# facebookresearch/LaViLa

Measured on AMD Instinct MI355X. Metric: clip-text pairs/s (whole node), TSF-B/16 4x224^2 + CLIP text tower, fwd+loss+bwd+AdamW (caption bound from the host tokens: INTEGRATION.md 1c one-line driver change; unmodified loop = config.device_readback), higher is better.
Workload: dtype bf16

## Files before the change

### include/lavila_hip.h

```cpp
#ifndef LAVILA_HIP_H
#define LAVILA_HIP_H

#include <stdint.h>

#ifdef __cplusplus
extern "C" {
#endif
#pragma GCC visibility push(default)

enum { LVL_F32 = 0, LVL_BF16 = 1 };
enum { LVL_OK = 0, LVL_EINVAL = -22, LVL_ENOSYS = -38, LVL_EHIP = -5 };
enum { LVL_ATTN_SPACE = 0, LVL_ATTN_TIME = 1, LVL_ATTN_CAUSAL = 2  };
enum { LVL_EPI_BIAS = 0, LVL_EPI_BIAS_QUICKGELU = 1, LVL_EPI_QUICKGELU_BWD = 2, LVL_EPI_BIAS_RESIDUAL = 3,
       LVL_EPI_BIAS_QUICKGELU_DERIV = 4, LVL_EPI_MUL_AUX_COLSUM = 5 };
enum { LVL_ACT_GELU_NEW = 0, LVL_ACT_SQRELU = 1 };

const char* lvl_version(void);
int lvl_debug_late_workgroups(int mod);
int lvl_set_compute_units(int n);
const char* lvl_last_error(void);
int64_t lvl_workspace_floats(const char* op, int64_t rows, int64_t cols);

int lvl_layernorm_fwd(const void* x, const void* x2, const float* xbias, const float* gamma,
                      const float* beta, void* s_out, void* y, float* mean, float* rstd,
                      int64_t rows, int cols, float eps, int dtype, void* stream);
int lvl_layernorm_bwd(const void* dy, const void* x, const void* x2, const float* xbias,
                      const float* gamma, const float* mean, const float* rstd, const void* dadd,
                      void* dx, void* dx_plain, float* dgamma, float* dbeta, float* dxsum, float* ws,
                      int64_t rows, int cols, int dtype, void* stream);

enum { LVL_LN_PLAIN = 1, LVL_LN_GENERAL = 2 };
int lvl_layernorm_fwd_mixed(const float* x, const void* x2, const float* xbias, const float* gamma,
                            const float* beta, float* s_out, void* y, float* mean, float* rstd,
                            int64_t rows, int cols, float eps, int flags, void* stream);
int lvl_layernorm_bwd_mixed(const void* dy, const float* x, const void* x2, const float* xbias,
                            const float* gamma, const float* mean, const float* rstd, const float* dadd,
                            float* dx, void* dx2, float* dgamma, float* dbeta, float* dxsum, float* ws,
                            int64_t rows, int cols, int flags, void* stream);

int lvl_droppath_add_layernorm_fwd(const void* res, const void* y, const float* ybias, const float* scale,
                                   const float* gamma, const float* beta, void* s_out, void* h_out, float* mean,
                                   float* rstd, int64_t rows, int64_t rows_per_sample, int cols, float eps,
                                   int dtype, void* stream);
int lvl_droppath_add_layernorm_bwd(const void* dh, const void* s, const float* gamma, const float* mean,
                                   const float* rstd, const float* scale, const void* dadd, void* ds, void* dy,
                                   float* dgamma, float* dbeta, float* dysum, float* ws, int64_t rows,
                                   int64_t rows_per_sample, int cols, int dtype, void* stream);

int lvl_layernorm_apply(const void* x, const void* x2, const float* xbias, const float* gamma,
                        const float* beta, const float* mean, const float* rstd, void* y,
                        int64_t rows, int cols, int dtype, void* stream);

int lvl_quickgelu_apply(const void* u, void* a, int64_t rows, int cols, int dtype, void* stream);

int lvl_bias_quickgelu_fwd(const void* u, const float* bias, void* a, int64_t rows, int cols,
                           int dtype, void* stream);
int lvl_bias_quickgelu_bwd(const void* da, const void* u, const float* bias, void* du, float* dbias,
                           float* ws, int64_t rows, int cols, int dtype, void* stream);

int lvl_patchify(const float* video, void* patches, int B, int C, int F, int H, int W, int P,
                 int frame_major, int dtype, void* stream);

int lvl_embed_tokens_fwd(const void* pe, const float* cls, const float* pos, const float* temporal,
                         void* x, int B, int F, int N, int D, int dtype, void* stream);
int64_t lvl_embed_tokens_bwd_ws(int F, int N, int D);
int lvl_embed_tokens_bwd(const void* dx, float* dpos, float* dtem, float* ws, int B, int F, int N, int D, int tem_rows,
                         int dtype, void* stream);

int lvl_text_embed_fwd(const int64_t* tokens, int64_t tok_stride, const float* table, const float* pos, void* x, int B,
                       int L, int W, int V, int dtype, void* stream);
int64_t lvl_text_embed_bwd_ws(int B, int L, int V);
int lvl_text_embed_bwd(const void* dx, const int64_t* tokens, int64_t tok_stride, float* dtable, float* dpos, int* ws,
                       int B, int L, int W, int V, int ctx, int dtype, void* stream);

int lvl_divided_attn_fwd(const void* qkv, void* out, float* lse, float* ws, int B, int F, int N,
                         int H, int mode, int dtype, void* stream);
int lvl_divided_attn_bwd(const void* qkv, const void* out, const void* dout, const float* lse,
                         void* dqkv, float* ws, int B, int F, int N, int H, int mode, int dtype,
                         void* stream);

int lvl_attention_fast_path(int mode, int F, int N, int H);
int lvl_attention_fast_path_f32(int mode, int F, int N, int H);
int lvl_debug_f32_generic(int on);
int lvl_debug_space_stream(int mode);
int lvl_debug_stream_variant(int v);
int lvl_set_fp8_qk(int on);
int lvl_debug_generic_attention_calls(int reset);

int lvl_causal_attn_fwd(const void* qkv, void* out, float* lse, int B, int L, int H, int dtype,
                        void* stream);
int lvl_causal_attn_bwd(const void* qkv, const void* out, const void* dout, const float* lse,
                        void* dqkv, float* ws, int B, int L, int H, int dtype, void* stream);

int lvl_clip_loss_fwd(const void* img_all, const void* txt_all, const float* scale, int B, int G,
                      int E, int row0, float* stats, int32_t* argmax, float* logits, int dtype,
                      void* stream);
int lvl_clip_loss_bwd(const void* img_all, const void* txt_all, const float* lse_all,
                      const float* scale, const float* upstream, float coef, int B, int G, int E,
                      int row0, int rows_only, float* dimg, float* dtxt, int dtype, void* stream);

int lvl_ssl_clip_loss_fwd(const void* img_all, const void* txt_all, const int32_t* ind_all,
                          const float* scales3, int B, int G, int E, int row0, float* stats,
                          int32_t* argmax, float* logits, int dtype, void* stream);
int lvl_ssl_clip_loss_bwd(const void* img_all, const void* txt_all, const int32_t* ind_all,
                          const float* lse_all, const float* scales3, const float* upstream, float coef,
                          int B, int G, int E, int row0, float* dimg, float* dtxt, int dtype,
                          void* stream);

int lvl_margin_loss_prepare(const void* img_all, const void* txt_all, const float* weight, float margin, int G,
                            int E, float* prep, int dtype, void* stream);
int lvl_margin_loss_fwd(const void* img_all, const void* txt_all, const float* prep, int B, int G, int E,
                        int row0, int with_diag, float* hinge, int32_t* count, int dtype, void* stream);
int lvl_margin_loss_bwd(const void* img_all, const void* txt_all, const float* prep, const float* upstream,
                        float coef, int B, int G, int E, int row0, float* dimg, float* dtxt, int dtype,
                        void* stream);

int lvl_token_xent_fwd(const void* logits, int64_t row_stride, const int64_t* labels, int64_t label_stride,
                       int64_t rows, int vocab, int64_t pad_id, float* lse, float* nll, int32_t* pred,
                       int32_t* correct, int32_t* counted, int dtype, void* stream);
int lvl_token_xent_reduce(const float* nll, const int32_t* correct, const int32_t* counted, int B, int T,
                          float* out3, void* stream);
int lvl_token_xent_bwd(const void* logits, int64_t row_stride, const int64_t* labels, int64_t label_stride,
                       const float* lse, const float* upstream, float coef, int64_t rows, int vocab, int64_t pad_id,
                       void* dlogits, int dtype, void* stream);

int lvl_cls_attn_fwd(const void* q, const void* kv, void* out, float* lse, int B, int T, int H, int dtype, void* stream);
int lvl_cls_attn_bwd(const void* q, const void* kv, const void* out, const void* dout, const float* lse, float* dq,
                     void* dkv, int B, int T, int H, int dtype, void* stream);

int lvl_mq_cross_attn_fwd(const void* q, int64_t q_batch_stride, const void* kv, void* out, int B, int NQ, int H,
                          int Tk, int dtype, void* stream);
int64_t lvl_mq_cross_attn_bwd_ws(int B, int NQ, int H, int shared_q);
int lvl_mq_cross_attn_bwd(const void* q, int64_t q_batch_stride, const void* kv, const void* dout, void* dq, void* dkv,
                          float* ws, int B, int NQ, int H, int Tk, int dtype, void* stream);

int lvl_linear_skinny(const void* x, const void* w, const float* bias, void* y, int M, int N, int K, int act, void* stream);
int lvl_linear_skinny_f32c(const void* x3, const void* w3, const float* bias, float* y, int M, int N, int K3, int act,
                           void* stream);
int lvl_linear_skinny_ln(const void* res, const void* y, const float* gate, const float* gamma, const float* beta,
                         float eps, void* res_out, const void* w, const float* bias, void* out, int M, int N, int K,
                         int act, void* stream);
int lvl_gpt2_embed(const int64_t* ids, const void* wte, const void* wpe, const int* pos_dev, void* out, int rows, int L,
                   int D, int vocab, int positions, int dtype, void* stream);
int lvl_gated_add_layernorm(const void* res, const void* y, const float* gate, const float* gamma, const float* beta,
                            float eps, void* sum_out, void* h_out, int rows, int D, int dtype, void* stream);
int lvl_act_inplace(void* u, int64_t n, int act, int dtype, void* stream);
int lvl_decode_self_attn(const void* qkv, void* cache, const int* pos_dev, void* out, int B, int Tcap, int H, int dtype,
                         void* stream);
int lvl_cross_attn_rows_fwd(const void* q, const void* kv, void* out, int rows, int qrep, int Tk, int H, int dtype,
                            void* stream);
int lvl_gated_add_layernorm_train(const void* res, const void* y, const float* gate, const float* gamma,
                                  const float* beta, float eps, void* sum_out, void* h_out, float* mean, float* rstd,
                                  int rows, int D, int dtype, void* stream);
int lvl_gated_add_layernorm_bwd(const void* dh, const void* s, const void* y, const float* gate, const float* gamma,
                                const float* mean, const float* rstd, const void* dadd, void* ds, void* dy, float* dgamma,
                                float* dbeta, float* dgate, float* ws, int rows, int D, int dtype, void* stream);
int lvl_act_fwd(const void* u, void* a, int64_t n, int act, int dtype, void* stream);
int lvl_act_bwd(const void* u, const void* da, void* du, int64_t n, int act, int dtype, void* stream);
int lvl_cross_attn_rows_bwd(const void* q, const void* kv, const void* dout, void* dq, void* dkv, int rows, int qrep,
                            int Tk, int H, int dtype, void* stream);

int lvl_sample_max_vocab(void);
int lvl_sample_next_token(const void* logits, int64_t row_stride, int rows, int vocab, float temperature, int top_k,
                          float top_p, const float* uniform, const int64_t* target, int64_t pad_id, int64_t* next_token,
                          float* nll, float* counted, float* dbg, void* stream);

int lvl_linear_tn(const void* x, const void* w, const float* bias, void* y, void* aux_out, const void* aux_in,
                  float* colsum, float* ws, uint32_t* sched, int64_t M, int N, int K, int epilogue, int dtype,
                  void* stream);

int lvl_linear_wgrad(const void* dy, const void* x, float* dw, float* dbias, float* ws, uint32_t* sched, int64_t M,
                     int N, int K, int dtype, void* stream);

int lvl_qkv_bias_grad(const void* dqkv, const void* dout, float* dbias, float* ws, int64_t rows, int D, int dtype,
                      void* stream);
int64_t lvl_divided_attn_bwd_bias_ws(int B, int F, int N, int H, int mode, int dtype);
int lvl_divided_attn_bwd_bias(const void* qkv, const void* out, const void* dout, const float* lse, void* dqkv, float* ws,
                              const float* dout_colsum, float* dbias, float* ws2, int B, int F, int N, int H, int mode,
                              int dtype, void* stream);
int lvl_debug_time_bwd_rider(int mode);
int lvl_vec_mat_f32(const float* v, const float* W, float* out, int N, int K, void* stream);

int lvl_cast_transpose(const float* src, void* dst, void* dst_t, int N, int K, void* stream);
int lvl_cast_transpose_multi(const void* desc, int count, int64_t total_tiles, void* stream);

int lvl_split_bf16x3(const float* src, void* dst, int64_t rows, int cols, int64_t src_row_stride,
                     int64_t dst_row_stride, int64_t dst_term_stride, int role, void* stream);

#pragma GCC visibility pop
#ifdef __cplusplus
}
#endif
#endif
```

### lavila_amd/_cabi.py

```python
import ctypes
import os
import threading

import torch

_HERE = os.path.dirname(os.path.abspath(__file__))
LIB_PATH = os.path.join(_HERE, 'lib', 'liblavila_hip.so')

LVL_F32, LVL_BF16 = 0, 1
ATTN_SPACE, ATTN_TIME = 0, 1
EPI_BIAS, EPI_BIAS_QUICKGELU, EPI_QUICKGELU_BWD, EPI_BIAS_RESIDUAL, EPI_BIAS_QUICKGELU_DERIV, EPI_MUL_AUX_COLSUM = 0, 1, 2, 3, 4, 5
LN_PLAIN, LN_GENERAL = 1, 2
ACT_GELU_NEW, ACT_SQRELU = 0, 1

_c = ctypes
_P, _I, _L, _F = _c.c_void_p, _c.c_int, _c.c_int64, _c.c_float

SIGNATURES = {
    'lvl_version': (_c.c_char_p, []),
    'lvl_set_compute_units': (_I, [_I]),
    'lvl_debug_late_workgroups': (_I, [_I]),
    'lvl_last_error': (_c.c_char_p, []),
    'lvl_workspace_floats': (_L, [_c.c_char_p, _L, _L]),
    'lvl_layernorm_fwd': (_I, [_P, _P, _P, _P, _P, _P, _P, _P, _P, _L, _I, _F, _I, _P]),
    'lvl_layernorm_bwd': (_I, [_P, _P, _P, _P, _P, _P, _P, _P, _P, _P, _P, _P, _P, _P, _L, _I, _I, _P]),
    'lvl_layernorm_fwd_mixed': (_I, [_P, _P, _P, _P, _P, _P, _P, _P, _P, _L, _I, _F, _I, _P]),
    'lvl_layernorm_bwd_mixed': (_I, [_P, _P, _P, _P, _P, _P, _P, _P, _P, _P, _P, _P, _P, _P, _L, _I, _I, _P]),
    'lvl_droppath_add_layernorm_fwd': (_I, [_P] * 10 + [_L, _L, _I, _F, _I, _P]),
    'lvl_droppath_add_layernorm_bwd': (_I, [_P] * 13 + [_L, _L, _I, _I, _P]),
    'lvl_layernorm_apply': (_I, [_P, _P, _P, _P, _P, _P, _P, _P, _L, _I, _I, _P]),
    'lvl_quickgelu_apply': (_I, [_P, _P, _L, _I, _I, _P]),
    'lvl_bias_quickgelu_fwd': (_I, [_P, _P, _P, _L, _I, _I, _P]),
    'lvl_bias_quickgelu_bwd': (_I, [_P, _P, _P, _P, _P, _P, _L, _I, _I, _P]),
    'lvl_patchify': (_I, [_P, _P, _I, _I, _I, _I, _I, _I, _I, _I, _P]),
    'lvl_embed_tokens_fwd': (_I, [_P, _P, _P, _P, _P, _I, _I, _I, _I, _I, _P]),
    'lvl_divided_attn_fwd': (_I, [_P, _P, _P, _P, _I, _I, _I, _I, _I, _I, _P]),
    'lvl_divided_attn_bwd': (_I, [_P, _P, _P, _P, _P, _P, _I, _I, _I, _I, _I, _I, _P]),
    'lvl_attention_fast_path': (_I, [_I, _I, _I, _I]),
    'lvl_attention_fast_path_f32': (_I, [_I, _I, _I, _I]),
    'lvl_debug_f32_generic': (_I, [_I]),
    'lvl_debug_space_stream': (_I, [_I]),
    'lvl_debug_stream_variant': (_I, [_I]),
    'lvl_set_fp8_qk': (_I, [_I]),
    'lvl_debug_generic_attention_calls': (_I, [_I]),
    'lvl_causal_attn_fwd': (_I, [_P, _P, _P, _I, _I, _I, _I, _P]),
    'lvl_causal_attn_bwd': (_I, [_P, _P, _P, _P, _P, _P, _I, _I, _I, _I, _P]),
    'lvl_clip_loss_fwd': (_I, [_P, _P, _P, _I, _I, _I, _I, _P, _P, _P, _I, _P]),
    'lvl_clip_loss_bwd': (_I, [_P, _P, _P, _P, _P, _F, _I, _I, _I, _I, _I, _P, _P, _I, _P]),
    'lvl_ssl_clip_loss_fwd': (_I, [_P, _P, _P, _P, _I, _I, _I, _I, _P, _P, _P, _I, _P]),
    'lvl_ssl_clip_loss_bwd': (_I, [_P, _P, _P, _P, _P, _P, _F, _I, _I, _I, _I, _P, _P, _I, _P]),
    'lvl_margin_loss_prepare': (_I, [_P, _P, _P, _F, _I, _I, _P, _I, _P]),
    'lvl_margin_loss_fwd': (_I, [_P, _P, _P, _I, _I, _I, _I, _I, _P, _P, _I, _P]),
    'lvl_margin_loss_bwd': (_I, [_P, _P, _P, _P, _F, _I, _I, _I, _I, _P, _P, _I, _P]),
    'lvl_token_xent_fwd': (_I, [_P, _L, _P, _L, _L, _I, _L, _P, _P, _P, _P, _P, _I, _P]),
    'lvl_token_xent_reduce': (_I, [_P, _P, _P, _I, _I, _P, _P]),
    'lvl_token_xent_bwd': (_I, [_P, _L, _P, _L, _P, _P, _F, _L, _I, _L, _P, _I, _P]),
    'lvl_linear_tn': (_I, [_P, _P, _P, _P, _P, _P, _P, _P, _P, _L, _I, _I, _I, _I, _P]),
    'lvl_linear_wgrad': (_I, [_P, _P, _P, _P, _P, _P, _L, _I, _I, _I, _P]),
    'lvl_cast_transpose': (_I, [_P, _P, _P, _I, _I, _P]),
    'lvl_cast_transpose_multi': (_I, [_P, _I, _L, _P]),
    'lvl_split_bf16x3': (_I, [_P, _P, _L, _I, _L, _L, _L, _I, _P]),
    'lvl_cls_attn_fwd': (_I, [_P, _P, _P, _P, _I, _I, _I, _I, _P]),
    'lvl_cls_attn_bwd': (_I, [_P, _P, _P, _P, _P, _P, _P, _I, _I, _I, _I, _P]),
    'lvl_mq_cross_attn_fwd': (_I, [_P, _L, _P, _P, _I, _I, _I, _I, _I, _P]),
    'lvl_mq_cross_attn_bwd_ws': (_L, [_I, _I, _I, _I]),
    'lvl_mq_cross_attn_bwd': (_I, [_P, _L, _P, _P, _P, _P, _P, _I, _I, _I, _I, _I, _P]),
    'lvl_qkv_bias_grad': (_I, [_P, _P, _P, _P, _L, _I, _I, _P]),
    'lvl_divided_attn_bwd_bias_ws': (_L, [_I, _I, _I, _I, _I, _I]),
    'lvl_divided_attn_bwd_bias': (_I, [_P, _P, _P, _P, _P, _P, _P, _P, _P, _I, _I, _I, _I, _I, _I, _P]),
    'lvl_vec_mat_f32': (_I, [_P, _P, _P, _I, _I, _P]),
    'lvl_embed_tokens_bwd_ws': (_L, [_I, _I, _I]),
    'lvl_embed_tokens_bwd': (_I, [_P, _P, _P, _P, _I, _I, _I, _I, _I, _I, _P]),
    'lvl_text_embed_fwd': (_I, [_P, _L, _P, _P, _P, _I, _I, _I, _I, _I, _P]),
    'lvl_text_embed_bwd_ws': (_L, [_I, _I, _I]),
    'lvl_text_embed_bwd': (_I, [_P, _P, _L, _P, _P, _P, _I, _I, _I, _I, _I, _I, _P]),
    'lvl_debug_time_bwd_rider': (_I, [_I]),
    'lvl_linear_skinny': (_I, [_P, _P, _P, _P, _I, _I, _I, _I, _P]),
    'lvl_linear_skinny_f32c': (_I, [_P, _P, _P, _P, _I, _I, _I, _I, _P]),
    'lvl_linear_skinny_ln': (_I, [_P, _P, _P, _P, _P, _F, _P, _P, _P, _P, _I, _I, _I, _I, _P]),
    'lvl_sample_max_vocab': (_I, []),
    'lvl_sample_next_token': (_I, [_P, _L, _I, _I, _F, _I, _F, _P, _P, _L, _P, _P, _P, _P, _P]),
    'lvl_gpt2_embed': (_I, [_P, _P, _P, _P, _P, _I, _I, _I, _I, _I, _I, _P]),
    'lvl_gated_add_layernorm': (_I, [_P, _P, _P, _P, _P, _F, _P, _P, _I, _I, _I, _P]),
    'lvl_act_inplace': (_I, [_P, _L, _I, _I, _P]),
    'lvl_gated_add_layernorm_train': (_I, [_P, _P, _P, _P, _P, _F, _P, _P, _P, _P, _I, _I, _I, _P]),
    'lvl_gated_add_layernorm_bwd': (_I, [_P] * 14 + [_I, _I, _I, _P]),
    'lvl_act_fwd': (_I, [_P, _P, _L, _I, _I, _P]),
    'lvl_act_bwd': (_I, [_P, _P, _P, _L, _I, _I, _P]),
    'lvl_cross_attn_rows_bwd': (_I, [_P, _P, _P, _P, _P, _I, _I, _I, _I, _I, _P]),
    'lvl_decode_self_attn': (_I, [_P, _P, _P, _P, _I, _I, _I, _I, _P]),
    'lvl_cross_attn_rows_fwd': (_I, [_P, _P, _P, _I, _I, _I, _I, _I, _P]),
}

_lib = None
_lock = threading.Lock()


class HipExtensionError(RuntimeError):
    pass


def lib():
    global _lib
    if _lib is not None:
        return _lib
    with _lock:
        if _lib is None:
            if not os.path.exists(LIB_PATH):
                raise HipExtensionError(
                    f'{LIB_PATH} is missing: build it with `python -m lavila_amd.build` '
                    '(or __graft_entry__.build()); lavila_amd has no CPU / eager fallback')
            try:
                handle = ctypes.CDLL(LIB_PATH)
            except OSError as e:
                raise HipExtensionError(f'cannot load {LIB_PATH}: {e}') from e
            for name, (res, args) in SIGNATURES.items():
                fn = getattr(handle, name)
                fn.restype = res
                fn.argtypes = args
            cus = os.environ.get('LAVILA_COMPUTE_UNITS')
            if cus and handle.lvl_set_compute_units(int(cus)) != 0:
                raise HipExtensionError('LAVILA_COMPUTE_UNITS: ' + handle.lvl_last_error().decode(errors='replace'))
            _lib = handle
    return _lib


def check(rc, what):
    if rc != 0:
        msg = lib().lvl_last_error().decode(errors='replace')
        raise HipExtensionError(f'{what} failed (status {rc}): {msg}')


def dtype_code(t: torch.Tensor) -> int:
    if t.dtype == torch.float32:
        return LVL_F32
    if t.dtype == torch.bfloat16:
        return LVL_BF16
    raise HipExtensionError(
        f'lavila_amd kernels take float32 or bfloat16 activations, got {t.dtype} '
        '(fp16 autocast is remapped to bf16 by the model wrappers; see INTEGRATION.md)')


def require_device(*tensors):
    cur = None
    for t in tensors:
        if t is None:
            continue
        if t.is_cuda:
            if cur is None:
                cur = torch.cuda.current_device()
            if t.device.index != cur:
                raise HipExtensionError(
                    f'lavila_amd: tensor on {t.device} but the current device is cuda:{cur}; call '
                    'torch.cuda.set_device() (one process per GPU) before running the model')
        if not t.is_cuda:
            raise HipExtensionError(
                'lavila_amd: tensor on %s -- the HIP kernels need a ROCm device tensor; there is no CPU '
                'fallback (the CPU oracle under oracle/ is test infrastructure only)' % t.device)
        if not t.is_contiguous():
            raise HipExtensionError('lavila_amd: non-contiguous tensor passed to a HIP kernel')


def ptr(t):
    return None if t is None else ctypes.c_void_p(t.data_ptr())


def stream_ptr():
    return ctypes.c_void_p(torch.cuda.current_stream().cuda_stream)


def workspace(op: str, rows: int, cols: int, device) -> torch.Tensor:
    n = lib().lvl_workspace_floats(op.encode(), rows, cols)
    if n < 0:
        raise HipExtensionError(f'unknown workspace op {op}')
    return torch.empty(max(int(n), 1), dtype=torch.float32, device=device)
```

### lavila_amd/csrc/gemm_tn_mfma.hip

```cpp
#include <type_traits>

#include "common.h"

int lvl_debug_late_mod();
int lvl_colsum_mid_rows();
int lvl_launch_column_reduce(const float* part, int nparts, int width, int seg, float* mid, float* out0, float* out1,
                             float* out2, hipStream_t st);

#pragma clang diagnostic ignored "-Winline-asm"

typedef __attribute__((ext_vector_type(8))) __bf16 gm_bf16x8;
typedef __attribute__((ext_vector_type(16))) float gm_f32x16;

namespace {

constexpr int BK = 64;
constexpr int TM = 256, TN = 256;
constexpr int SLOT = 128 * 128;
constexpr int NSLOT = 8;
constexpr int BIAS_OFF = NSLOT * SLOT;
constexpr int MBOX_OFF = BIAS_OFF + 4 * 1024;
constexpr int SMEM_B = MBOX_OFF + 64;
constexpr int DYN_MIN_NB = 5;
enum { S_X0 = 0, S_X1 = 1, S_W0 = 2, S_W1 = 3 };

__device__ __forceinline__ gm_f32x16 mfma32(uint4 a, uint4 b, gm_f32x16 c) {
  return __builtin_amdgcn_mfma_f32_32x32x16_bf16(__builtin_bit_cast(gm_bf16x8, a), __builtin_bit_cast(gm_bf16x8, b),
                                                 c, 0, 0, 0);
}

__device__ __forceinline__ float quick_gelu_grad(float u) {
  const float s = sigmoid1702(u);
  return s * (1.f + 1.702f * u * (1.f - s));
}

__device__ __forceinline__ float qgelu_grad1(float y, float r) { return fmaf((1.f - r) * y, 1.702f, r); }

__device__ __forceinline__ uint4 widen_pair(uint2 a, uint2 b) {
  const auto r0 = __builtin_amdgcn_permlane32_swap(a.x, b.x, false, false);
  const auto r1 = __builtin_amdgcn_permlane32_swap(a.y, b.y, false, false);
  return make_uint4(r0[0], r1[0], r0[1], r1[1]);
}

__device__ __forceinline__ void gm_store16(void* p, uint4 v) { *reinterpret_cast<uint4*>(p) = v; }

#ifdef GM_AUDIT
#define GM_AUD_STORE(j) (gm_aud_st += 1u << (8 * (j)))
#define GM_AUD_COLPART() (++gm_aud_cp)
constexpr int GM_AUDIT_CAP = 255;
__device__ __forceinline__ int gm_wave_max(int v) {
#pragma unroll
  for (int m = 32; m >= 1; m >>= 1) v = max(v, __shfl_xor(v, m, 64));
  return v;
}
#else
#define GM_AUD_STORE(j) ((void)0)
#define GM_AUD_COLPART() ((void)0)
#endif

template <int EPI, bool F32O>
__global__ __launch_bounds__(512) void gemm_tn_kernel(const uint16_t* __restrict__ X, const uint16_t* __restrict__ W,
                                                      const float* __restrict__ bias, void* __restrict__ Yv,
                                                      void* __restrict__ aux_out_v,
                                                      const void* __restrict__ aux_in_v,
                                                      float* __restrict__ colpart, int64_t M, int N, int K,
                                                      int tiles_n, int ntiles, unsigned* __restrict__ sched,
                                                      int late_mod) {
  using out_t = std::conditional_t<F32O, float, uint16_t>;
  out_t* __restrict__ const Y = static_cast<out_t*>(Yv);
  out_t* __restrict__ const aux_out = static_cast<out_t*>(aux_out_v);
  const out_t* __restrict__ const aux_in = static_cast<const out_t*>(aux_in_v);
  extern __shared__ __attribute__((aligned(1024))) uint8_t smem[];
  const int tid = threadIdx.x, lane = tid & 63;
  const int wave = __builtin_amdgcn_readfirstlane(tid >> 6);
  const int wm = wave >> 2, wn = wave & 3;
  const int nb = K / BK;
  const int nx = gridDim.x >= 8 ? 8 : 1;
  const int bid = blockIdx.x, xcd = bid % nx, wpx = gridDim.x / nx;
  const int tq = ntiles / nx, tr = ntiles % nx;
  const int cnt = tq + (xcd < tr ? 1 : 0);
  const int xstart = xcd < tr ? xcd * (tq + 1) : tr * (tq + 1) + (xcd - tr) * tq;
  const bool dyn = sched != nullptr;
  if (dyn) __builtin_assume(nb >= DYN_MIN_NB);
  if (!dyn && bid / nx >= cnt) return;
  int my_tiles = dyn ? 0x7fffffff : (cnt - bid / nx + wpx - 1) / wpx;
  int pair_even = xstart + bid / nx, pair_odd = pair_even;
  auto set_pair = [&](int i, int v) { if (i & 1) pair_odd = v; else pair_even = v; };
  auto get_pair = [&](int i) { return (i & 1) ? pair_odd : pair_even; };
  uint32_t pend = 0;
  unsigned* const ctr = sched + xcd;
  uint64_t exec_save;
  auto pull = [&]() {
    if (wave == 0)
      asm volatile("s_mov_b64 %1, exec\n\ts_mov_b64 exec, 1\n\tglobal_atomic_add %0, %2, %3, %4 sc0\n\ts_mov_b64 exec, %1"
                   : "=v"(pend), "=&s"(exec_save) : "v"(0u), "v"(1u), "s"(ctr) : "memory");
  };
  auto publish = [&]() {
    if (wave == 0)
      asm volatile("s_mov_b64 %0, exec\n\ts_mov_b64 exec, 1\n\tds_write_b32 %1, %2\n\ts_mov_b64 exec, %0"
                   : "=&s"(exec_save) : "v"((uint32_t)(uintptr_t)smem + MBOX_OFF), "v"(pend) : "memory");
  };
  auto mailbox = [&]() -> int {
    uint32_t v;
    asm volatile("ds_read_b32 %0, %1\n\ts_waitcnt lgkmcnt(0)" : "=v"(v) : "v"((uint32_t)(uintptr_t)smem + MBOX_OFF) : "memory");
    return __builtin_amdgcn_readfirstlane(v);
  };
  const bool late = dyn && late_mod > 0 && bid % late_mod == 1;
  if (dyn && !late) pull();

  auto decode_tile = [&](int pair, int& tm, int& tn) {
    tm = pair / tiles_n;
    tn = pair - tm * tiles_n;
  };

  uint32_t xrel[4], wrel[2], xclamp;
  {
    const int sub = lane >> 3;
    const int chunk = (lane & 7) ^ ((4 * wave + (sub >> 1)) & 7);
#pragma unroll
    for (int h = 0; h < 2; ++h) {
      const int lr = 8 * (wave + 8 * h) + sub;
#pragma unroll
      for (int q = 0; q < 2; ++q) xrel[q * 2 + h] = (uint32_t)(q * 128 + lr) * (uint32_t)(K * 2) + chunk * 16;
      wrel[h] = (uint32_t)((lr >> 5) * 64 + (lr & 31)) * (uint32_t)(K * 2) + chunk * 16;
    }
    xclamp = (uint32_t)((M - 1) * K * 2) + chunk * 16;
  }
  const uint32_t lds0 = (uint32_t)(uintptr_t)smem;
  int f_i = 0, f_j = 0;
  uint32_t f_xrow;
  const char* f_wbase;
  auto fetch_tile = [&](int i) {
    if (!dyn) set_pair(i, xstart + bid / nx + i * wpx);
    const int pair = __builtin_amdgcn_readfirstlane(get_pair(i));
    int tm, tn;
    decode_tile(pair, tm, tn);
    f_xrow = (uint32_t)tm * (uint32_t)(TM * K * 2);
    f_wbase = reinterpret_cast<const char*>(W) + (int64_t)tn * TN * K * 2;
    if (EPI != 2 && bias != nullptr && wave == 0) {
      const uint32_t m0v = __builtin_amdgcn_readfirstlane(lds0 + BIAS_OFF + (uint32_t)(i & 3) * 1024);
      const uint32_t off = (uint32_t)lane * 16;
      const char* base = reinterpret_cast<const char*>(bias + tn * TN);
      asm volatile("s_mov_b32 m0, %0\n\ts_nop 0\n\tglobal_load_lds_dwordx4 %1, %2" ::"s"(m0v), "v"(off), "s"(base)
                   : "memory", "m0");
    }
  };
  auto fetch_advance = [&]() {
    if (++f_j == nb) {
      if (dyn && f_i + 1 < my_tiles) {
        const int v = mailbox();
        if (v < cnt) {
          set_pair(f_i + 1, xstart + v);
        } else {
          my_tiles = f_i + 1;
        }
      }
      if (f_i + 1 < my_tiles) {
        f_j = 0;
        fetch_tile(++f_i);
      } else {
        f_j = nb - 1;
      }
    }
  };
  auto issue_fill = [&](int type, int par, int h) {
    const char* base = type < S_W0 ? reinterpret_cast<const char*>(X) + (int64_t)f_j * (BK * 2)
                                   : f_wbase + (int64_t)f_j * (BK * 2) + (type == S_W1 ? (int64_t)32 * K * 2 : 0);
    uint32_t off;
    if (type < S_W0) {
      off = xrel[type * 2 + h] + f_xrow;
      off = off < xclamp ? off : xclamp;
    } else {
      off = wrel[h];
    }
    const uint32_t m0v =
// ... 285 lines not shown
#ifdef GM_AUDIT
  int* const audit = reinterpret_cast<int*>(colpart + ((EPI == 2 || EPI == 5) ? (size_t)2 * (ntiles / tiles_n) * N : 0)) +
                     ((size_t)bid * 8 + wave) * (1 + GM_AUDIT_CAP) * 4;
  int aud_n = 0, aud_rec[4] = {0, 0, 0, 0};
#endif
  if (late) {
    my_tiles = 0;
  } else if (dyn) {
    asm volatile("s_waitcnt vmcnt(0)" ::: "memory");
    publish();
    asm volatile("s_waitcnt lgkmcnt(0)" ::: "memory");
    __builtin_amdgcn_s_barrier();
    const int v = mailbox();
    if (v >= cnt) my_tiles = 0;
    pair_even = xstart + v;
    __builtin_amdgcn_s_barrier();
    if (my_tiles) pull();
  }
  GM_STAMP();
  if (my_tiles > 0) {
  fetch_tile(0);
#pragma unroll
  for (int b0 = 0; b0 < 2; ++b0) {
    issue_group(S_X0, b0 * 4);
    issue_group(S_W0, b0 * 4);
    issue_group(S_W1, b0 * 4);
    issue_group(S_X1, b0 * 4);
    fetch_advance();
  }
#define GM_BAR(N)                                                     \
  do {                                                                \
    asm volatile("s_waitcnt vmcnt(%0)" ::"n"(N) : "memory");          \
    __builtin_amdgcn_s_barrier();                                     \
    asm volatile("" ::: "memory");                                    \
    __builtin_amdgcn_sched_barrier(0);                                \
  } while (0)
#define GM_PHASE(xf, wf, c, rd, dm)                                                                       \
  do {                                                                                                    \
    _Pragma("unroll") for (int kk = 0; kk < 4; ++kk) {                                                    \
      _Pragma("unroll") for (int mt = 0; mt < 2; ++mt) {                                                  \
        c[mt] = mfma32(wf[kk], xf[mt * 4 + kk], c[mt]);                                                   \
        __builtin_amdgcn_sched_barrier(0);                                                                \
        rd(kk * 2 + mt);                                                                                  \
        dm(kk * 2 + mt);                                                                                  \
        __builtin_amdgcn_sched_barrier(0);                                                                \
      }                                                                                                   \
    }                                                                                                     \
  } while (0)
  GM_BAR(12);
  read_x(S_X0, xA);
  read_w(S_W0, wA);
  __builtin_amdgcn_sched_barrier(0);
  GM_STAMP();
  init_acc(0);
  constexpr int NS = F32O ? 0 : (EPI == 1 || EPI == 4 ? 32 : 16);
  auto k_block = [&](auto a0_, auto a1_) {
    constexpr int A0 = decltype(a0_)::value, A1 = decltype(a1_)::value;
    const uint8_t* sb = smem + par * SLOT;
    const uint8_t* sbn = smem + (par ^ 4) * SLOT;
    auto rd_w1 = [&](int k) { if (k < 4) wB[k] = *reinterpret_cast<const uint4*>(sb + S_W1 * SLOT + wa[k]); };
    auto rd_x1 = [&](int k) { xB[k] = *reinterpret_cast<const uint4*>(sb + S_X1 * SLOT + xa[k & 3] + (k >> 2) * 4096); };
    auto rd_x0 = [&](int k) { xA[k] = *reinterpret_cast<const uint4*>(sbn + S_X0 * SLOT + xa[k & 3] + (k >> 2) * 4096); };
    auto rd_w0 = [&](int k) { if (k & 1) wA[k >> 1] = *reinterpret_cast<const uint4*>(sbn + S_W0 * SLOT + wa[k >> 1]); };
    auto dm_none = [&](int) {};
    auto dm_x0w0 = [&](int k) {
      if (k == 0) issue_fill(S_X0, par, 0);
      if (k == 2) issue_fill(S_X0, par, 1);
      if (k == 4) issue_fill(S_W0, par, 0);
      if (k == 6) issue_fill(S_W0, par, 1);
    };
    auto dm_w1 = [&](int k) {
      if (k == 1) issue_fill(S_W1, par, 0);
      if (k == 5) issue_fill(S_W1, par, 1);
    };
    auto dm_x1 = [&](int k) {
      if (k == 0) issue_fill(S_X1, par, 0);
      if (k == 4) issue_fill(S_X1, par, 1);
    };
    GM_BAR(10 + A0);
    GM_PHASE(xA, wA, acc[0][0], rd_w1, dm_none);
    GM_BAR(8 + A0);
    GM_PHASE(xA, wB, acc[0][1], rd_x1, dm_x0w0);
    GM_BAR(10 + A1);
    GM_PHASE(xB, wB, acc[1][1], rd_x0, dm_w1);
    GM_BAR(10 + A1);
    GM_PHASE(xB, wA, acc[1][0], rd_w0, dm_x1);
    fetch_advance();
    par ^= 4;
  };
  using I0 = std::integral_constant<int, 0>;
  using IS = std::integral_constant<int, NS>;
  for (int i = 0; i < my_tiles; ++i) {
    int j = 0;
    if (i > 0) {
#ifdef GM_AUDIT
      if (lane == 0 && aud_n < GM_AUDIT_CAP) {
#pragma unroll
        for (int q = 0; q < 4; ++q) audit[4 * (1 + aud_n) + q] = aud_rec[q];
      }
      ++aud_n;
#endif
      k_block(IS{}, IS{});
      if (nb > 1) k_block(IS{}, I0{});
      j = 2;
    }
    for (; j < nb; ++j) {
      if (dyn && j == 2) {
        if (wave == 0) asm volatile("s_waitcnt vmcnt(10)" ::: "memory");
        publish();
      }
      k_block(I0{}, I0{});
    }
    GM_STAMP();
    if (dyn && my_tiles == 0x7fffffff) pull();
    const int pair = get_pair(i);
    int tm, tn;
    decode_tile(pair, tm, tn);
    epilogue(tm, tn, i);
    const bool tail = NS > 0 && __builtin_amdgcn_readfirstlane((int64_t)tm * TM + TM > M ? 1 : 0);
    if (tail) asm volatile("s_waitcnt vmcnt(0)" ::: "memory");
#ifdef GM_AUDIT
    {
      int issued = gm_wave_max((int)gm_aud_cp);
#pragma unroll
      for (int q = 0; q < 4; ++q) issued += gm_wave_max((int)((gm_aud_st >> (8 * q)) & 255u));
      aud_rec[0] = tm;
      aud_rec[1] = tn;
      aud_rec[2] = issued;
      aud_rec[3] = tail ? 0 : NS;
      gm_aud_st = gm_aud_cp = 0;
    }
#endif
    GM_STAMP();
    init_acc(i + 1);
    __builtin_amdgcn_sched_barrier(0);
  }
  }
#undef GM_BAR
#undef GM_PHASE
  asm volatile("s_waitcnt vmcnt(0)" ::: "memory");
#ifdef GM_AUDIT
  if (lane == 0) audit[0] = aud_n;
#endif
  asm volatile("" ::"v"(pend));
  if (dyn && wave == 0 && lane == 0) {
    const unsigned gone = __hip_atomic_fetch_add(sched + 8, 1u, __ATOMIC_RELAXED, __HIP_MEMORY_SCOPE_AGENT);
    if (gone == gridDim.x - 1) {
#pragma unroll
      for (int q = 0; q < 9; ++q) __hip_atomic_store(sched + q, 0u, __ATOMIC_RELAXED, __HIP_MEMORY_SCOPE_AGENT);
    }
  }
}

int num_cus() { return lvl_persistent_cus(); }

template <int EPI, bool F32O = false>
int launch_tn(const void* x, const void* w, const float* bias, void* y, void* aux_out, const void* aux_in,
              float* colpart, int64_t M, int N, int K, unsigned* sched, hipStream_t st) {
  constexpr int shmem = SMEM_B;
  const int rc = lvl_allow_lds<gemm_tn_kernel<EPI, F32O>>();
  if (rc != LVL_OK) return rc;
  const int tiles_n = N / TN;
  const int64_t tiles_m = (M + TM - 1) / TM;
  const int64_t ntiles = tiles_m * tiles_n;
  if (ntiles > 0x7fffffff) return lvl_fail(LVL_EINVAL, "linear_tn: too many tiles");
  int grid = (int)(ntiles < num_cus() ? ntiles : num_cus());
  if (grid >= 8) grid -= grid % 8;
  if (K / BK < DYN_MIN_NB) sched = nullptr;
  hipLaunchKernelGGL((gemm_tn_kernel<EPI, F32O>), dim3((unsigned)grid), dim3(512), shmem, st, (const uint16_t*)x,
                     (const uint16_t*)w, bias, y, aux_out, aux_in, colpart, M,
                     N, K, tiles_n, (int)ntiles, sched, sched ? lvl_debug_late_mod() : 0);
  LVL_CHECK_LAUNCH("linear_tn");
  return LVL_OK;
}

}

int64_t lvl_linear_tn_workspace_floats(int64_t M, int64_t N) {
  return (2 * ((M + TM - 1) / TM) + lvl_colsum_mid_rows()) * N;
}

#ifdef GM_TRACE
extern "C" int lvl_linear_tn_trace(const void* x, const void* w, const float* bias, void* y, void* trace, int64_t M,
                                   int N, int K, void* stream) {
  return launch_tn<0>(x, w, bias, y, nullptr, nullptr, (float*)trace, M, N, K, nullptr, (hipStream_t)stream);
}
extern "C" int lvl_linear_tn_trace_epi(const void* x, const void* w, const float* bias, void* y, void* aux_out,
                                       const void* aux_in, void* trace, int64_t M, int N, int K, int epilogue, void* stream) {
  hipStream_t st = (hipStream_t)stream;
  switch (epilogue) {
    case 0: return launch_tn<0>(x, w, bias, y, nullptr, nullptr, (float*)trace, M, N, K, nullptr, st);
    case 1: return launch_tn<1>(x, w, bias, y, aux_out, nullptr, (float*)trace, M, N, K, nullptr, st);
    case 3: return launch_tn<3>(x, w, bias, y, nullptr, aux_in, (float*)trace, M, N, K, nullptr, st);
    case 4: return launch_tn<4>(x, w, bias, y, aux_out, nullptr, (float*)trace, M, N, K, nullptr, st);
    case 5: return launch_tn<5>(x, w, nullptr, y, nullptr, aux_in, (float*)trace, M, N, K, nullptr, st);
  }
  return -1;
}
#endif

#ifdef GM_AUDIT
extern "C" int lvl_linear_tn_audit_cap() { return GM_AUDIT_CAP; }
extern "C" int lvl_linear_tn_audit(const void* x, const void* w, const float* bias, void* y, void* aux_out,
                                   const void* aux_in, void* audit, uint32_t* sched, int64_t M, int N, int K, int epilogue,
                                   int dtype, void* stream) {
  hipStream_t st = (hipStream_t)stream;
  float* a = (float*)audit;
  if (dtype == LVL_F32) {
    switch (epilogue) {
      case 0: return launch_tn<0, true>(x, w, bias, y, nullptr, nullptr, a, M, N, K, sched, st);
      case 1: return launch_tn<1, true>(x, w, bias, y, aux_out, nullptr, a, M, N, K, sched, st);
      case 2: return launch_tn<2, true>(x, w, nullptr, y, nullptr, aux_in, a, M, N, K, sched, st);
      case 3: return launch_tn<3, true>(x, w, bias, y, nullptr, aux_in, a, M, N, K, sched, st);
    }
    return -1;
  }
  switch (epilogue) {
    case 0: return launch_tn<0>(x, w, bias, y, nullptr, nullptr, a, M, N, K, sched, st);
    case 1: return launch_tn<1>(x, w, bias, y, aux_out, nullptr, a, M, N, K, sched, st);
    case 2: return launch_tn<2>(x, w, nullptr, y, nullptr, aux_in, a, M, N, K, sched, st);
    case 3: return launch_tn<3>(x, w, bias, y, nullptr, aux_in, a, M, N, K, sched, st);
    case 4: return launch_tn<4>(x, w, bias, y, aux_out, nullptr, a, M, N, K, sched, st);
    case 5: return launch_tn<5>(x, w, nullptr, y, nullptr, aux_in, a, M, N, K, sched, st);
  }
  return -1;
}
#endif

extern "C" int lvl_linear_tn(const void* x, const void* w, const float* bias, void* y, void* aux_out,
                             const void* aux_in, float* colsum, float* ws, uint32_t* sched, int64_t M, int N, int K,
                             int epilogue, int dtype, void* stream) {
  LVL_REQUIRE(x && w && y, "linear_tn: null pointer");
  LVL_REQUIRE(dtype == LVL_BF16 || dtype == LVL_F32, "linear_tn: unknown dtype %d", dtype);
  LVL_REQUIRE(M > 0 && N > 0 && K > 0, "linear_tn: empty problem");
  if (N % TN != 0 || K % BK != 0)
    return lvl_fail(LVL_ENOSYS, "linear_tn: no tiling for N=%d K=%d (N %% 256 == 0 and K %% 64 == 0 needed)", N, K);
  if ((uint64_t)M * K * 2 >= (1ull << 32) || (uint64_t)N * K * 2 >= (1ull << 32))
    return lvl_fail(LVL_ENOSYS, "linear_tn: operand larger than 4 GiB (32-bit DMA offsets)");
  LVL_REQUIRE(lvl_aligned16(x) && lvl_aligned16(w) && lvl_aligned16(y) && lvl_aligned16(bias) &&
                  lvl_aligned16(aux_out) && lvl_aligned16(aux_in),
              "linear_tn: pointers must be 16-byte aligned");
  hipStream_t st = (hipStream_t)stream;
  if (dtype == LVL_F32) {
    LVL_REQUIRE(K % (3 * BK) == 0, "linear_tn (f32 class): K = %d is not 3 x a multiple of 64", K);
    switch (epilogue) {
      case LVL_EPI_BIAS:
        return launch_tn<0, true>(x, w, bias, y, nullptr, nullptr, nullptr, M, N, K, sched, st);
      case LVL_EPI_BIAS_QUICKGELU:
        LVL_REQUIRE(aux_out != nullptr, "linear_tn: the QuickGELU epilogue writes the pre-activation to aux_out");
        return launch_tn<1, true>(x, w, bias, y, aux_out, nullptr, nullptr, M, N, K, sched, st);
      case LVL_EPI_BIAS_RESIDUAL:
        LVL_REQUIRE(aux_in != nullptr, "linear_tn: the residual epilogue reads the residual rows from aux_in");
        return launch_tn<3, true>(x, w, bias, y, nullptr, aux_in, nullptr, M, N, K, sched, st);
      case LVL_EPI_QUICKGELU_BWD: {
        LVL_REQUIRE(aux_in != nullptr && colsum != nullptr && ws != nullptr && lvl_aligned16(ws),
                    "linear_tn: the QuickGELU-backward epilogue needs aux_in, colsum and a workspace");
        const int rc = launch_tn<2, true>(x, w, nullptr, y, nullptr, aux_in, ws, M, N, K, sched, st);
        if (rc != LVL_OK) return rc;
        const int P = (int)(2 * ((M + TM - 1) / TM));
        return lvl_launch_column_reduce(ws, P, N, N, ws + (size_t)P * N, colsum, nullptr, nullptr, st);
      }
      case LVL_EPI_BIAS_QUICKGELU_DERIV:
      case LVL_EPI_MUL_AUX_COLSUM:
        return lvl_fail(LVL_ENOSYS, "linear_tn: epilogue %d is a bf16 epilogue (the f32-class mode keeps the pre-activation: "
                                    "LVL_EPI_BIAS_QUICKGELU / LVL_EPI_QUICKGELU_BWD)", epilogue);
      default:
        return lvl_fail(LVL_EINVAL, "linear_tn: unknown epilogue %d", epilogue);
    }
  }
  switch (epilogue) {
    case LVL_EPI_BIAS:
      return launch_tn<0>(x, w, bias, y, nullptr, nullptr, nullptr, M, N, K, sched, st);
    case LVL_EPI_BIAS_QUICKGELU:
      LVL_REQUIRE(aux_out != nullptr, "linear_tn: the QuickGELU epilogue writes the pre-activation to aux_out");
      return launch_tn<1>(x, w, bias, y, aux_out, nullptr, nullptr, M, N, K, sched, st);
    case LVL_EPI_BIAS_RESIDUAL:
      LVL_REQUIRE(aux_in != nullptr, "linear_tn: the residual epilogue reads the residual rows from aux_in");
      return launch_tn<3>(x, w, bias, y, nullptr, aux_in, nullptr, M, N, K, sched, st);
    case LVL_EPI_QUICKGELU_BWD: {
      LVL_REQUIRE(aux_in != nullptr && colsum != nullptr && ws != nullptr && lvl_aligned16(ws),
                  "linear_tn: the QuickGELU-backward epilogue needs aux_in, colsum and a workspace");
      const int rc = launch_tn<2>(x, w, nullptr, y, nullptr, aux_in, ws, M, N, K, sched, st);
      if (rc != LVL_OK) return rc;
      const int P = (int)(2 * ((M + TM - 1) / TM));
      return lvl_launch_column_reduce(ws, P, N, N, ws + (size_t)P * N, colsum, nullptr, nullptr, st);
    }
    case LVL_EPI_BIAS_QUICKGELU_DERIV:
      LVL_REQUIRE(aux_out != nullptr, "linear_tn: the QuickGELU + derivative epilogue writes quickgelu'(u) to aux_out");
      return launch_tn<4>(x, w, bias, y, aux_out, nullptr, nullptr, M, N, K, sched, st);
    case LVL_EPI_MUL_AUX_COLSUM: {
      LVL_REQUIRE(aux_in != nullptr && colsum != nullptr && ws != nullptr && lvl_aligned16(ws),
                  "linear_tn: the multiply-by-aux epilogue needs aux_in, colsum and a workspace");
      const int rc = launch_tn<5>(x, w, nullptr, y, nullptr, aux_in, ws, M, N, K, sched, st);
      if (rc != LVL_OK) return rc;
      const int P = (int)(2 * ((M + TM - 1) / TM));
      return lvl_launch_column_reduce(ws, P, N, N, ws + (size_t)P * N, colsum, nullptr, nullptr, st);
    }
    default:
      return lvl_fail(LVL_EINVAL, "linear_tn: unknown epilogue %d", epilogue);
  }
}
```

Before: 1558.

## Split tail GEMM tiles into quarter sub-tiles to fill idle CUs

Adds a 128x128 sub-tile GEMM kernel for the bias and residual bf16 epilogues, plus a planner that runs full tiles on the persistent kernel and splits the last partial wave (or tiny problems) into four sub-tiles each, so more compute units stay busy. It also splits short-K problems with more tiles than CUs into row chunks of separate launches. The cost is extra kernel launches and lower per-workgroup reuse in the sub-tile path. A plan query entry point is exported.

```diff
diff --git a/include/lavila_hip.h b/include/lavila_hip.h
--- a/include/lavila_hip.h
+++ b/include/lavila_hip.h
@@ -168,6 +168,7 @@
 int lvl_linear_tn(const void* x, const void* w, const float* bias, void* y, void* aux_out, const void* aux_in,
                   float* colsum, float* ws, uint32_t* sched, int64_t M, int N, int K, int epilogue, int dtype,
                   void* stream);
+int lvl_linear_tn_plan(int64_t M, int N, int K, int epilogue, int dtype, int* out);
 
 int lvl_linear_wgrad(const void* dy, const void* x, float* dw, float* dbias, float* ws, uint32_t* sched, int64_t M,
                      int N, int K, int dtype, void* stream);
diff --git a/lavila_amd/_cabi.py b/lavila_amd/_cabi.py
--- a/lavila_amd/_cabi.py
+++ b/lavila_amd/_cabi.py
@@ -56,6 +56,7 @@
     'lvl_token_xent_reduce': (_I, [_P, _P, _P, _I, _I, _P, _P]),
     'lvl_token_xent_bwd': (_I, [_P, _L, _P, _L, _P, _P, _F, _L, _I, _L, _P, _I, _P]),
     'lvl_linear_tn': (_I, [_P, _P, _P, _P, _P, _P, _P, _P, _P, _L, _I, _I, _I, _I, _P]),
+    'lvl_linear_tn_plan': (_I, [_L, _I, _I, _I, _I, _P]),
     'lvl_linear_wgrad': (_I, [_P, _P, _P, _P, _P, _P, _L, _I, _I, _I, _P]),
     'lvl_cast_transpose': (_I, [_P, _P, _P, _I, _I, _P]),
     'lvl_cast_transpose_multi': (_I, [_P, _I, _L, _P]),
diff --git a/lavila_amd/csrc/gemm_tn_mfma.hip b/lavila_amd/csrc/gemm_tn_mfma.hip
--- a/lavila_amd/csrc/gemm_tn_mfma.hip
+++ b/lavila_amd/csrc/gemm_tn_mfma.hip
@@ -21,6 +21,7 @@
 constexpr int BIAS_OFF = NSLOT * SLOT;
 constexpr int MBOX_OFF = BIAS_OFF + 4 * 1024;
 constexpr int SMEM_B = MBOX_OFF + 64;
+constexpr int MULTI_TILE_MIN_NB = 3;
 constexpr int DYN_MIN_NB = 5;
 enum { S_X0 = 0, S_X1 = 1, S_W0 = 2, S_W1 = 3 };
 
@@ -612,25 +613,221 @@
   }
 }
 
+constexpr int SUB = 128;
+constexpr int SUB_SMEM_B = 4 * SLOT;
+constexpr int SUB_FILLS = 4;
+
+template <int EPI>
+__global__ __launch_bounds__(512) __attribute__((amdgpu_waves_per_eu(4))) void gemm_tn_sub_kernel(
+    const uint16_t* __restrict__ X, const uint16_t* __restrict__ W, const float* __restrict__ bias, uint16_t* __restrict__ Y,
+    const uint16_t* __restrict__ aux_in, int64_t M, int N, int K, int tiles_n, int tile0) {
+  static_assert(EPI == 0 || EPI == 3, "sub-tile kernel: plain and residual epilogues only");
+  extern __shared__ __attribute__((aligned(1024))) uint8_t smem[];
+  const int tid = threadIdx.x, lane = tid & 63;
+  const int wave = __builtin_amdgcn_readfirstlane(tid >> 6);
+  const int wm = wave >> 2, wn = wave & 3;
+  const int r5 = lane & 31, hi = lane >> 5;
+  const int nb = K / BK;
+  const int tile = tile0 + (int)(blockIdx.x >> 2), quarter = blockIdx.x & 3;
+  const int tm = tile / tiles_n, tn = tile - tm * tiles_n;
+  const int64_t m0 = (int64_t)tm * TM + (quarter >> 1) * SUB;
+  const int n0 = tn * TN + (quarter & 1) * SUB;
+  if (m0 >= M) return;
+
+  gm_f32x16 acc[2];
+  if (bias != nullptr) {
+#pragma unroll
+    for (int rq = 0; rq < 4; ++rq) {
+      const float4 b = *reinterpret_cast<const float4*>(bias + n0 + wn * 32 + 8 * rq + 4 * hi);
+#pragma unroll
+      for (int mt = 0; mt < 2; ++mt) {
+        acc[mt][4 * rq + 0] = b.x;
+        acc[mt][4 * rq + 1] = b.y;
+        acc[mt][4 * rq + 2] = b.z;
+        acc[mt][4 * rq + 3] = b.w;
+      }
+    }
+  } else {
+#pragma unroll
+    for (int mt = 0; mt < 2; ++mt)
+#pragma unroll
+      for (int r = 0; r < 16; ++r) acc[mt][r] = 0.f;
+  }
+
+  uint32_t xoff[2], woff[2];
+  {
+    const int sub = lane >> 3;
+    const int chunk = (lane & 7) ^ ((4 * wave + (sub >> 1)) & 7);
+#pragma unroll
+    for (int h = 0; h < 2; ++h) {
+      const int lr = 8 * (wave + 8 * h) + sub;
+      const int64_t m = m0 + lr < M ? m0 + lr : M - 1;
+      xoff[h] = (uint32_t)(m * K * 2 + chunk * 16);
+      woff[h] = (uint32_t)(n0 + lr) * (uint32_t)(K * 2) + chunk * 16;
+    }
+  }
+  const uint32_t lds0 = (uint32_t)(uintptr_t)smem;
+  auto issue_block = [&](int j, int half) {
+    const char* xb = reinterpret_cast<const char*>(X) + (int64_t)j * (BK * 2);
+    const char* wb = reinterpret_cast<const char*>(W) + (int64_t)j * (BK * 2);
+#pragma unroll
+    for (int t = 0; t < 2; ++t)
+#pragma unroll
+      for (int h = 0; h < 2; ++h) {
+        const uint32_t m0v =
+            __builtin_amdgcn_readfirstlane(lds0 + (uint32_t)(half * 2 + t) * SLOT + (uint32_t)(wave + 8 * h) * 1024);
+        asm volatile("s_mov_b32 m0, %0\n\ts_nop 0\n\tglobal_load_lds_dwordx4 %1, %2" ::"s"(m0v),
+                     "v"(t == 0 ? xoff[h] : woff[h]), "s"(t == 0 ? xb : wb)
+                     : "memory", "m0");
+      }
+  };
+  uint32_t xa[4], wa[4];
+#pragma unroll
+  for (int kk = 0; kk < 4; ++kk) {
+    const int offk = ((2 * kk + hi) ^ ((r5 >> 1) & 7)) * 16;
+    xa[kk] = (uint32_t)((wm * 64 + r5) * 128 + offk);
+    wa[kk] = (uint32_t)((wn * 32 + r5) * 128 + offk);
+  }
+
+  issue_block(0, 0);
+  if (nb > 1) issue_block(1, 1);
+  for (int j = 0; j < nb; ++j) {
+    if (j + 1 < nb) {
+      asm volatile("s_waitcnt vmcnt(%0)" ::"n"(SUB_FILLS) : "memory");
+    } else {
+      asm volatile("s_waitcnt vmcnt(0)" ::: "memory");
+    }
+    __builtin_amdgcn_s_barrier();
+    asm volatile("" ::: "memory");
+    const uint8_t* sx = smem + (j & 1) * (2 * SLOT);
+    const uint8_t* sw = sx + SLOT;
+    uint4 xf[2][4], wf[4];
+#pragma unroll
+    for (int kk = 0; kk < 4; ++kk) {
+      wf[kk] = *reinterpret_cast<const uint4*>(sw + wa[kk]);
+#pragma unroll
+      for (int mt = 0; mt < 2; ++mt) xf[mt][kk] = *reinterpret_cast<const uint4*>(sx + xa[kk] + mt * 4096);
+    }
+    asm volatile("s_waitcnt lgkmcnt(0)" ::: "memory");
+    __builtin_amdgcn_s_barrier();
+    if (j + 2 < nb) issue_block(j + 2, j & 1);
+#pragma unroll
+    for (int kk = 0; kk < 4; ++kk)
+#pragma unroll
+      for (int mt = 0; mt < 2; ++mt) acc[mt] = mfma32(wf[kk], xf[mt][kk], acc[mt]);
+  }
+
+  uint2 ub[EPI == 3 ? 2 : 1][4];
+  if constexpr (EPI == 3) {
+#pragma unroll
+    for (int mt = 0; mt < 2; ++mt) {
+      const int64_t m = m0 + wm * 64 + mt * 32 + r5;
+      const uint16_t* urow = aux_in + (m < M ? m : M - 1) * (int64_t)N + n0 + wn * 32 + 4 * hi;
+#pragma unroll
+      for (int rq = 0; rq < 4; ++rq) ub[mt][rq] = *reinterpret_cast<const uint2*>(urow + 8 * rq);
+    }
+  }
+#pragma unroll
+  for (int mt = 0; mt < 2; ++mt) {
+    uint2 ypk[4];
+#pragma unroll
+    for (int rq = 0; rq < 4; ++rq) {
+      float v[4];
+#pragma unroll
+      for (int e = 0; e < 4; ++e) v[e] = acc[mt][4 * rq + e];
+      if constexpr (EPI == 3) {
+        const uint2 ab = ub[mt][rq];
+        const float a4[4] = {bf16_lo(ab.x), bf16_hi(ab.x), bf16_lo(ab.y), bf16_hi(ab.y)};
+#pragma unroll
+        for (int e = 0; e < 4; ++e) v[e] += a4[e];
+      }
+      ypk[rq] = make_uint2(f32x2_to_bf16x2(v[0], v[1]), f32x2_to_bf16x2(v[2], v[3]));
+    }
+    uint4 y4[2];
+#pragma unroll
+    for (int jj = 0; jj < 2; ++jj) y4[jj] = widen_pair(ypk[2 * jj], ypk[2 * jj + 1]);
+    const int64_t m = m0 + wm * 64 + mt * 32 + r5;
+    if (m < M) {
+#pragma unroll
+      for (int jj = 0; jj < 2; ++jj) gm_store16(Y + m * (int64_t)N + n0 + wn * 32 + 16 * jj + 8 * hi, y4[jj]);
+    }
+  }
+}
+
 int num_cus() { return lvl_persistent_cus(); }
 
 template <int EPI, bool F32O = false>
 int launch_tn(const void* x, const void* w, const float* bias, void* y, void* aux_out, const void* aux_in,
-              float* colpart, int64_t M, int N, int K, unsigned* sched, hipStream_t st) {
+              float* colpart, int64_t M, int N, int K, unsigned* sched, hipStream_t st, int64_t main_tiles = -1) {
   constexpr int shmem = SMEM_B;
   const int rc = lvl_allow_lds<gemm_tn_kernel<EPI, F32O>>();
   if (rc != LVL_OK) return rc;
   const int tiles_n = N / TN;
   const int64_t tiles_m = (M + TM - 1) / TM;
-  const int64_t ntiles = tiles_m * tiles_n;
+  const int64_t ntiles = main_tiles >= 0 ? main_tiles : tiles_m * tiles_n;
   if (ntiles > 0x7fffffff) return lvl_fail(LVL_EINVAL, "linear_tn: too many tiles");
   int grid = (int)(ntiles < num_cus() ? ntiles : num_cus());
   if (grid >= 8) grid -= grid % 8;
+  if (K / BK < MULTI_TILE_MIN_NB && ntiles > grid) {
+    if (main_tiles >= 0 || tiles_n > grid)
+      return lvl_fail(LVL_ENOSYS, "linear_tn: K = %d (< %d) needs N / 256 = %d <= %d compute units", K, MULTI_TILE_MIN_NB * BK,
+                      tiles_n, grid);
+    constexpr int64_t osz = F32O ? 4 : 2;
+    const int64_t rows = (int64_t)(grid / tiles_n) * TM;
+    for (int64_t r0 = 0; r0 < M; r0 += rows) {
+      auto at = [&](const void* p, int64_t bytes) { return p ? static_cast<const char*>(p) + bytes : nullptr; };
+      const int rc2 = launch_tn<EPI, F32O>(at(x, r0 * K * 2), w, bias, const_cast<char*>(at(y, r0 * N * osz)),
+                                           const_cast<char*>(at(aux_out, r0 * N * osz)), at(aux_in, r0 * N * osz),
+                                           colpart ? colpart + 2 * (r0 / TM) * N : nullptr, M - r0 < rows ? M - r0 : rows, N,
+                                           K, nullptr, st);
+      if (rc2 != LVL_OK) return rc2;
+    }
+    return LVL_OK;
+  }
   if (K / BK < DYN_MIN_NB) sched = nullptr;
   hipLaunchKernelGGL((gemm_tn_kernel<EPI, F32O>), dim3((unsigned)grid), dim3(512), shmem, st, (const uint16_t*)x,
                      (const uint16_t*)w, bias, y, aux_out, aux_in, colpart, M,
                      N, K, tiles_n, (int)ntiles, sched, sched ? lvl_debug_late_mod() : 0);
   LVL_CHECK_LAUNCH("linear_tn");
+  return LVL_OK;
+}
+
+struct TnPlan {
+  int64_t main_tiles;
+  int sub_wgs;
+  int cus;
+};
+TnPlan plan_tn(int64_t M, int N, int K, int epilogue, int dtype) {
+  const int64_t ntiles = ((M + TM - 1) / TM) * (N / TN);
+  int c = num_cus();
+  if (c >= 8) c -= c % 8;
+  TnPlan p{ntiles, 0, c};
+  if (dtype != LVL_BF16 || (epilogue != LVL_EPI_BIAS && epilogue != LVL_EPI_BIAS_RESIDUAL)) return p;
+  const int64_t R = ntiles / c, L = ntiles % c;
+  if (4 * ntiles <= c) {
+    p.main_tiles = 0;
+    p.sub_wgs = (int)(4 * ntiles);
+  } else if (R >= 1 && L > 0 && 4 * L <= c && (R == 1 || K / BK >= MULTI_TILE_MIN_NB)) {
+    p.main_tiles = R * c;
+    p.sub_wgs = (int)(4 * L);
+  }
+  return p;
+}
+
+template <int EPI>
+int launch_tn_planned(const void* x, const void* w, const float* bias, void* y, const void* aux_in, int64_t M, int N, int K,
+                      unsigned* sched, hipStream_t st) {
+  const TnPlan p = plan_tn(M, N, K, EPI, LVL_BF16);
+  if (p.sub_wgs == 0) return launch_tn<EPI>(x, w, bias, y, nullptr, aux_in, nullptr, M, N, K, sched, st);
+  if (p.main_tiles > 0) {
+    const int rc = launch_tn<EPI>(x, w, bias, y, nullptr, aux_in, nullptr, M, N, K, sched, st, p.main_tiles);
+    if (rc != LVL_OK) return rc;
+  }
+  const int rc = lvl_allow_lds<gemm_tn_sub_kernel<EPI>>();
+  if (rc != LVL_OK) return rc;
+  hipLaunchKernelGGL((gemm_tn_sub_kernel<EPI>), dim3((unsigned)p.sub_wgs), dim3(512), SUB_SMEM_B, st, (const uint16_t*)x,
+                     (const uint16_t*)w, bias, (uint16_t*)y, (const uint16_t*)aux_in, M, N, K, N / TN, (int)p.main_tiles);
+  LVL_CHECK_LAUNCH("linear_tn (sub-tiles)");
   return LVL_OK;
 }
 
@@ -686,6 +883,20 @@
   return -1;
 }
 #endif
+
+extern "C" int lvl_linear_tn_plan(int64_t M, int N, int K, int epilogue, int dtype, int* out) {
+  LVL_REQUIRE(out != nullptr, "linear_tn_plan: null pointer");
+  LVL_REQUIRE(dtype == LVL_BF16 || dtype == LVL_F32, "linear_tn_plan: unknown dtype %d", dtype);
+  LVL_REQUIRE(M > 0 && N > 0 && K > 0, "linear_tn_plan: empty problem");
+  if (N % TN != 0 || K % BK != 0)
+    return lvl_fail(LVL_ENOSYS, "linear_tn_plan: no tiling for N=%d K=%d (N %% 256 == 0 and K %% 64 == 0 needed)", N, K);
+  const TnPlan p = plan_tn(M, N, K, epilogue, dtype);
+  if (p.main_tiles > 0x7fffffff) return lvl_fail(LVL_EINVAL, "linear_tn_plan: too many tiles");
+  out[0] = (int)p.main_tiles;
+  out[1] = p.sub_wgs;
+  out[2] = p.cus;
+  return LVL_OK;
+}
 
 extern "C" int lvl_linear_tn(const void* x, const void* w, const float* bias, void* y, void* aux_out,
                              const void* aux_in, float* colsum, float* ws, uint32_t* sched, int64_t M, int N, int K,
@@ -730,13 +941,13 @@
   }
   switch (epilogue) {
     case LVL_EPI_BIAS:
-      return launch_tn<0>(x, w, bias, y, nullptr, nullptr, nullptr, M, N, K, sched, st);
+      return launch_tn_planned<0>(x, w, bias, y, nullptr, M, N, K, sched, st);
     case LVL_EPI_BIAS_QUICKGELU:
       LVL_REQUIRE(aux_out != nullptr, "linear_tn: the QuickGELU epilogue writes the pre-activation to aux_out");
       return launch_tn<1>(x, w, bias, y, aux_out, nullptr, nullptr, M, N, K, sched, st);
     case LVL_EPI_BIAS_RESIDUAL:
       LVL_REQUIRE(aux_in != nullptr, "linear_tn: the residual epilogue reads the residual rows from aux_in");
-      return launch_tn<3>(x, w, bias, y, nullptr, aux_in, nullptr, M, N, K, sched, st);
+      return launch_tn_planned<3>(x, w, bias, y, aux_in, M, N, K, sched, st);
     case LVL_EPI_QUICKGELU_BWD: {
       LVL_REQUIRE(aux_in != nullptr && colsum != nullptr && ws != nullptr && lvl_aligned16(ws),
                   "linear_tn: the QuickGELU-backward epilogue needs aux_in, colsum and a workspace");
```

Result: no change. 1562, median of 6 (+0.2%).
